# bogus2000/anytime-3D-reconstruction

Hardware: AMD Instinct MI355X
Metric: 32^3 voxel reconstructions/sec at batch=256; IoU delta vs reference (higher is better)
Workload: dtype bf16

## Files before the change

anytime-3d-reconstruction_amd/csrc/conv_direct.hip:

```cpp
#include "direct_common.h"

namespace {

constexpr int CD_CIN = 64, CD_COUT = 128;
constexpr int CD_RB = CD_CIN * 2;
constexpr int CD_PIECES = 51;
constexpr int CD_TILE = CD_PIECES * 1024;
constexpr int CD_WST = CD_COUT * 128;
constexpr int CD_NST = 3;
constexpr int CD_RING = 2 * CD_TILE;
constexpr int CD_DUMMY = CD_RING + CD_NST * CD_WST;
constexpr int CD_LDS = CD_DUMMY + 1024;
constexpr int CD_SP = CD_COUT * 2 + 16;

__global__ __launch_bounds__(512, 1) void conv_direct_kernel(const __bf16 *__restrict__ x, const __bf16 *__restrict__ w,
                                                             const float *__restrict__ scale, const float *__restrict__ shift,
                                                             void *__restrict__ y, int dout_log2, unsigned x_bytes, unsigned w_bytes,
                                                             int act, int out_fp8) {
    extern __shared__ __attribute__((aligned(16))) char smem[];
    const int tid = threadIdx.x, lane = tid & 63;
    const int wave = __builtin_amdgcn_readfirstlane(tid >> 6);
    const int wm = wave >> 1, wn = wave & 1;
    const int lo = dout_log2, no = 1 << lo, li = lo + 1, n = 1 << li;

    const VvDirectBox box = vv_direct_box(no);
    const int b = box.b, od0 = box.od0, oh0 = box.oh0, ow0 = box.ow0;

    const u32x4 rsx = vv_make_rsrc(x, x_bytes), rsw = vv_make_rsrc(w, w_bytes);
    const unsigned lds0 = (unsigned)(unsigned long long)(lptr_t)smem;

    auto issue_x = [&](int q, int slot) {
        const int piece = slot * 8 + wave;
        const int rl = piece * 8 + (lane >> 3);
        const int zd = rl / 81, rem = rl - zd * 81, jh = rem / 9, jw = rem - jh * 9;
        const int g = (lane & 7) ^ (jw & 7);
        const int id = 2 * (od0 + zd) + ((q >> 2) & 1) - 1, ih = 2 * (oh0 + jh) + ((q >> 1) & 1) - 1, iw = 2 * (ow0 + jw) + (q & 1) - 1;
// ... 156 lines not shown
    auto issue_w = [&](int c) {
        const int q = c >> 3, a = c & 7;
        const int td = 2 * ((a >> 2) & 1) + ((q >> 2) & 1), th = 2 * ((a >> 1) & 1) + ((q >> 1) & 1), tw = 2 * (a & 1) + (q & 1);
        const int t = (td * 4 + th) * 4 + tw;
        const unsigned st = lds0 + CD_RING + (c % CD_NST) * CD_WST;
#pragma unroll
        for (int i = 0; i < 2; ++i) {
            const int row = (wave * 2 + i) * 8 + (lane >> 3);
            const int g = (lane & 7) ^ ((row >> 1) & 7);
            const unsigned vo = c < 64 ? (unsigned)row * (64 * CD_RB) + t * CD_RB + g * 16 : 0xFFFFFFF0u;
            vv_dma16(rsw, vo, st + (wave * 2 + i) * 1024);
        }
    };

#pragma unroll 1
    for (int s = 0; s < 7; ++s) issue_x(0, s);
    issue_w(0);
    issue_w(1);
    issue_w(2);
    vv_wait_vm<0>();
    __syncthreads();

    const int r = lane & 15, kq = lane >> 4;
    const int rl0 = wm * 81 + (r >> 3) * 9 + (r & 7);
    unsigned xo[2][2], wo[2];
#pragma unroll
    for (int aw = 0; aw < 2; ++aw)
#pragma unroll
        for (int ks = 0; ks < 2; ++ks) xo[aw][ks] = lds0 + rl0 * CD_RB + (((ks * 4 + kq) ^ ((2 * ((r & 7) + aw)) & 7)) << 4);
#pragma unroll
    for (int ks = 0; ks < 2; ++ks) wo[ks] = lds0 + CD_RING + (wn * 64 + r) * 128 + (((ks * 4 + kq) ^ ((r >> 1) & 7)) << 4);

    f32x4 acc[4][4];
#pragma unroll
    for (int i = 0; i < 4; ++i)
#pragma unroll
        for (int j = 0; j < 4; ++j) acc[i][j] = f32x4{0.f, 0.f, 0.f, 0.f};

#define CD16_LD(F, XA, XOFF, WA)                                                                                                    \
    asm volatile("ds_read_b128 %0, %8 offset:%10\n\tds_read_b128 %1, %8 offset:%11\n\tds_read_b128 %2, %8 offset:%12\n\t"         \
                 "ds_read_b128 %3, %8 offset:%13\n\tds_read_b128 %4, %9\n\tds_read_b128 %5, %9 offset:2048\n\t"                   \
                 "ds_read_b128 %6, %9 offset:4096\n\tds_read_b128 %7, %9 offset:6144"                                               \
                 : "=&v"(F[0]), "=&v"(F[1]), "=&v"(F[2]), "=&v"(F[3]), "=&v"(F[4]), "=&v"(F[5]), "=&v"(F[6]), "=&v"(F[7])            \
                 : "v"(XA), "v"(WA), "n"(XOFF), "n"((XOFF) + 2304), "n"((XOFF) + 4608), "n"((XOFF) + 6912)                          \
                 : "memory")
#define CD16_WAIT(F, N)                                                                                                             \
    asm volatile("s_waitcnt lgkmcnt(%8)"                                                                                            \
                 : "+v"(F[0]), "+v"(F[1]), "+v"(F[2]), "+v"(F[3]), "+v"(F[4]), "+v"(F[5]), "+v"(F[6]), "+v"(F[7])                    \
                 : "n"(N)                                                                                                           \
                 : "memory")
#define CD16_SB __builtin_amdgcn_sched_barrier(0)
#define CD16_RD(D, A, OFF) asm volatile("ds_read_b128 %0, %1 offset:%2" : "=&v"(D) : "v"(A), "n"(OFF) : "memory")
#define CD16_MF(F, COT, CT)                                                                                                         \
    acc[COT][CT] = __builtin_amdgcn_mfma_f32_16x16x32_bf16(*reinterpret_cast<const bf16x8 *>(&F[4 + COT]),                          \
                                                           *reinterpret_cast<const bf16x8 *>(&F[CT]), acc[COT][CT], 0, 0, 0)

    u32x4 P[8], Q[8];
    CD16_LD(P, xo[0][0], 0, wo[0]);

#pragma unroll 1
    for (int q = 0; q < 8; ++q) {
        const unsigned tsel = (q & 1) * CD_TILE, tnext = ((q + 1) & 1) * CD_TILE;
        auto tap = [&](auto a_c) {
            constexpr int A = decltype(a_c)::value;
            constexpr int AW = A & 1, TO = (((A >> 2) & 1) * 81 + ((A >> 1) & 1) * 9 + AW) * CD_RB;
            constexpr int AN = (A + 1) & 7, AWN = AN & 1, TON = (((AN >> 2) & 1) * 81 + ((AN >> 1) & 1) * 9 + AWN) * CD_RB;
            const int c = q * 8 + A;
            const unsigned wsel = (c % CD_NST) * CD_WST, wnext = ((c + 1) % CD_NST) * CD_WST;
            const unsigned xq = xo[AW][1] + tsel, wq = wo[1] + wsel;
            CD16_WAIT(P, 0);
            CD16_SB;
            CD16_MF(P, 0, 0); CD16_MF(P, 0, 1); CD16_SB; CD16_RD(Q[0], xq, TO); CD16_RD(Q[4], wq, 0); CD16_SB;
            CD16_MF(P, 0, 2); CD16_MF(P, 0, 3); CD16_SB; CD16_RD(Q[1], xq, TO + 2304); CD16_RD(Q[5], wq, 2048); CD16_SB;
            CD16_MF(P, 1, 0); CD16_MF(P, 1, 1); CD16_SB; CD16_RD(Q[2], xq, TO + 4608); CD16_RD(Q[6], wq, 4096); CD16_SB;
            CD16_MF(P, 1, 2); CD16_MF(P, 1, 3); CD16_SB; CD16_RD(Q[3], xq, TO + 6912); CD16_RD(Q[7], wq, 6144); CD16_SB;
            CD16_MF(P, 2, 0); CD16_MF(P, 2, 1); CD16_MF(P, 2, 2); CD16_MF(P, 2, 3);
            CD16_MF(P, 3, 0); CD16_MF(P, 3, 1); CD16_MF(P, 3, 2); CD16_MF(P, 3, 3);
            CD16_SB;
            CD16_WAIT(Q, 0);
            vv_wait_vm<(A == 0 || A == 7) ? 2 : 3>();
            __syncthreads();
            CD16_SB;
            CD16_MF(Q, 0, 0); CD16_MF(Q, 0, 1);
            if (A < 7) issue_x(q + 1, A);
            CD16_MF(Q, 0, 2); CD16_MF(Q, 0, 3);
            issue_w(c + 3);
            const unsigned xp = xo[AWN][0] + (A == 7 ? tnext : tsel), wp = wo[0] + wnext;
            CD16_SB;
            CD16_MF(Q, 1, 0); CD16_MF(Q, 1, 1); CD16_SB; CD16_RD(P[0], xp, TON); CD16_RD(P[4], wp, 0); CD16_SB;
            CD16_MF(Q, 1, 2); CD16_MF(Q, 1, 3); CD16_SB; CD16_RD(P[1], xp, TON + 2304); CD16_RD(P[5], wp, 2048); CD16_SB;
            CD16_MF(Q, 2, 0); CD16_MF(Q, 2, 1); CD16_SB; CD16_RD(P[2], xp, TON + 4608); CD16_RD(P[6], wp, 4096); CD16_SB;
            CD16_MF(Q, 2, 2); CD16_MF(Q, 2, 3); CD16_SB; CD16_RD(P[3], xp, TON + 6912); CD16_RD(P[7], wp, 6144); CD16_SB;
            CD16_MF(Q, 3, 0); CD16_MF(Q, 3, 1); CD16_MF(Q, 3, 2); CD16_MF(Q, 3, 3);
            CD16_SB;
        };
        tap(std::integral_constant<int, 0>{});
        tap(std::integral_constant<int, 1>{});
        tap(std::integral_constant<int, 2>{});
        tap(std::integral_constant<int, 3>{});
        tap(std::integral_constant<int, 4>{});
        tap(std::integral_constant<int, 5>{});
        tap(std::integral_constant<int, 6>{});
        tap(std::integral_constant<int, 7>{});
    }
    CD16_WAIT(P, 0);
    vv_wait_vm<0>();
    __syncthreads();

    char *stage = smem;
    f32x4 scv[4], shv[4];
#pragma unroll
    for (int cot = 0; cot < 4; ++cot) { scv[cot] = f32x4{1.f, 1.f, 1.f, 1.f}; shv[cot] = f32x4{0.f, 0.f, 0.f, 0.f}; }
    if (scale) {
#pragma unroll
        for (int cot = 0; cot < 4; ++cot) scv[cot] = *reinterpret_cast<const f32x4 *>(scale + wn * 64 + cot * 16 + 4 * kq);
    }
    if (shift) {
#pragma unroll
        for (int cot = 0; cot < 4; ++cot) shv[cot] = *reinterpret_cast<const f32x4 *>(shift + wn * 64 + cot * 16 + 4 * kq);
    }
    auto fill = VV_DIRECT_FILL16(CD_SP, wn * 64);
    auto with_out = [&](auto act_c) {
        if (out_fp8) fill(act_c, std::true_type{});
        else fill(act_c, std::false_type{});
    };
    VV_WITH_ACT(act, with_out);
    __syncthreads();
    vv_direct_store_box<512, CD_SP, CD_COUT, CD_COUT>(stage, y, box, lo, tid, out_fp8);
}


constexpr int CDH_COUT = 64;
constexpr int CDH_WST = CDH_COUT * 128;
constexpr int CDH_RING = CD_TILE;
constexpr int CDH_DUMMY = CDH_RING + CD_NST * CDH_WST;
constexpr int CDH_LDS = CDH_DUMMY + 1024;
constexpr int CDH_SP = CDH_COUT * 2 + 16;

__global__ __launch_bounds__(256, 2) void conv_direct16h_kernel(const __bf16 *__restrict__ x, const __bf16 *__restrict__ w,
                                                                const float *__restrict__ scale, const float *__restrict__ shift,
                                                                void *__restrict__ y, int dout_log2, unsigned x_bytes, unsigned w_bytes,
                                                                int act, int out_fp8, int stagger, int abl) {
    extern __shared__ __attribute__((aligned(16))) char smem[];
    const int tid = threadIdx.x, lane = tid & 63;
// ... 50 lines not shown
    const int r = lane & 15, kq = lane >> 4;
    const int rl0 = wm * 81 + (r >> 3) * 9 + (r & 7);
    unsigned xo[2][2], wo[2];
#pragma unroll
    for (int aw = 0; aw < 2; ++aw)
#pragma unroll
        for (int ks = 0; ks < 2; ++ks) xo[aw][ks] = lds0 + rl0 * CD_RB + (((ks * 4 + kq) ^ ((2 * ((r & 7) + aw)) & 7)) << 4);
#pragma unroll
    for (int ks = 0; ks < 2; ++ks) wo[ks] = lds0 + CDH_RING + r * 128 + (((ks * 4 + kq) ^ ((r >> 1) & 7)) << 4);

    f32x4 acc[4][4];
#pragma unroll
    for (int i = 0; i < 4; ++i)
#pragma unroll
        for (int j = 0; j < 4; ++j) acc[i][j] = f32x4{0.f, 0.f, 0.f, 0.f};

    u32x4 P[8], Q[8];
#pragma unroll 1
    for (int q = 0; q < 8; ++q) {
        if (q > 0) {
            vv_wait_vm<0>();
            __syncthreads();
        }
        CD16_LD(P, xo[0][0], 0, wo[0] + ((q * 8) % CD_NST) * CDH_WST);
        auto tap = [&](auto a_c) {
            constexpr int A = decltype(a_c)::value;
            constexpr int AW = A & 1, TO = (((A >> 2) & 1) * 81 + ((A >> 1) & 1) * 9 + AW) * CD_RB;
            constexpr int AN = (A + 1) & 7, AWN = AN & 1, TON = (((AN >> 2) & 1) * 81 + ((AN >> 1) & 1) * 9 + AWN) * CD_RB;
            const int c = q * 8 + A;
            const unsigned wsel = (c % CD_NST) * CDH_WST, wnext = ((c + 1) % CD_NST) * CDH_WST;
            const unsigned xq = xo[AW][1], wq = wo[1] + wsel;
            CD16_WAIT(P, 0);
            CD16_SB;
            CD16_MF(P, 0, 0); CD16_MF(P, 0, 1); CD16_SB; CD16_RD(Q[0], xq, TO); CD16_RD(Q[4], wq, 0); CD16_SB;
            CD16_MF(P, 0, 2); CD16_MF(P, 0, 3); CD16_SB; CD16_RD(Q[1], xq, TO + 2304); CD16_RD(Q[5], wq, 2048); CD16_SB;
            CD16_MF(P, 1, 0); CD16_MF(P, 1, 1); CD16_SB; CD16_RD(Q[2], xq, TO + 4608); CD16_RD(Q[6], wq, 4096); CD16_SB;
            CD16_MF(P, 1, 2); CD16_MF(P, 1, 3); CD16_SB; CD16_RD(Q[3], xq, TO + 6912); CD16_RD(Q[7], wq, 6144); CD16_SB;
            CD16_MF(P, 2, 0); CD16_MF(P, 2, 1); CD16_MF(P, 2, 2); CD16_MF(P, 2, 3);
            CD16_MF(P, 3, 0); CD16_MF(P, 3, 1); CD16_MF(P, 3, 2); CD16_MF(P, 3, 3);
            CD16_SB;
            CD16_WAIT(Q, 0);
            vv_wait_vm<2>();
            __syncthreads();
            CD16_SB;
            CD16_MF(Q, 0, 0); CD16_MF(Q, 0, 1);
            CD16_MF(Q, 0, 2); CD16_MF(Q, 0, 3);
            issue_w(c + 3);
            CD16_SB;
            if (A < 7) {
                const unsigned xp = xo[AWN][0], wp = wo[0] + wnext;
                CD16_MF(Q, 1, 0); CD16_MF(Q, 1, 1); CD16_SB; CD16_RD(P[0], xp, TON); CD16_RD(P[4], wp, 0); CD16_SB;
                CD16_MF(Q, 1, 2); CD16_MF(Q, 1, 3); CD16_SB; CD16_RD(P[1], xp, TON + 2304); CD16_RD(P[5], wp, 2048); CD16_SB;
                CD16_MF(Q, 2, 0); CD16_MF(Q, 2, 1); CD16_SB; CD16_RD(P[2], xp, TON + 4608); CD16_RD(P[6], wp, 4096); CD16_SB;
                CD16_MF(Q, 2, 2); CD16_MF(Q, 2, 3); CD16_SB; CD16_RD(P[3], xp, TON + 6912); CD16_RD(P[7], wp, 6144); CD16_SB;
            } else {
                const bool more = q < 7 && !(abl & 1);
                CD16_MF(Q, 1, 0); CD16_MF(Q, 1, 1); CD16_SB;
                if (more) { issue_x(q + 1, 0); issue_x(q + 1, 1); issue_x(q + 1, 2); }
                CD16_SB; CD16_MF(Q, 1, 2); CD16_MF(Q, 1, 3); CD16_SB;
                if (more) { issue_x(q + 1, 3); issue_x(q + 1, 4); issue_x(q + 1, 5); }
                CD16_SB; CD16_MF(Q, 2, 0); CD16_MF(Q, 2, 1); CD16_SB;
                if (more) { issue_x(q + 1, 6); issue_x(q + 1, 7); issue_x(q + 1, 8); }
                CD16_SB; CD16_MF(Q, 2, 2); CD16_MF(Q, 2, 3); CD16_SB;
                if (more) { issue_x(q + 1, 9); issue_x(q + 1, 10); issue_x(q + 1, 11); issue_x(q + 1, 12); }
                CD16_SB;
            }
            CD16_MF(Q, 3, 0); CD16_MF(Q, 3, 1); CD16_MF(Q, 3, 2); CD16_MF(Q, 3, 3);
            CD16_SB;
        };
        tap(std::integral_constant<int, 0>{});
        tap(std::integral_constant<int, 1>{});
        tap(std::integral_constant<int, 2>{});
        tap(std::integral_constant<int, 3>{});
        tap(std::integral_constant<int, 4>{});
        tap(std::integral_constant<int, 5>{});
        tap(std::integral_constant<int, 6>{});
        tap(std::integral_constant<int, 7>{});
// ... 77 lines not shown
```

anytime-3d-reconstruction_amd/csrc/convt_whole.hip:

```cpp

#include <utility>

#include "common.h"

namespace {

constexpr int CW_X = 512 * 256;
constexpr int CW_WST = 64 * 128;
constexpr int CW_NST = 3;
constexpr int CW_RING = CW_X;
constexpr int CW_ZERO = CW_RING + CW_NST * CW_WST;
constexpr int CW_SS = CW_ZERO + 256;
constexpr int CW_LDS = CW_SS + 512;

#define CW_LD(F, X0, X1, WA)                                                                                                     \
    asm volatile("ds_read_b128 %0, %4\n\tds_read_b128 %1, %5\n\tds_read_b128 %2, %6\n\tds_read_b128 %3, %6 offset:4096"          \
                 : "=&v"(F[0]), "=&v"(F[1]), "=&v"(F[2]), "=&v"(F[3])                                                            \
                 : "v"(X0), "v"(X1), "v"(WA)                                                                                     \
                 : "memory")
#define CW_WAIT(F, N) asm volatile("s_waitcnt lgkmcnt(%4)" : "+v"(F[0]), "+v"(F[1]), "+v"(F[2]), "+v"(F[3]) : "n"(N) : "memory")
#define CW_MFMA4(F)                                                                                                              \
    do {                                                                                                                         \
        _Pragma("unroll") for (int nt = 0; nt < 2; ++nt) _Pragma("unroll") for (int mt = 0; mt < 2; ++mt)                        \
            acc[nt][mt] = __builtin_amdgcn_mfma_f32_32x32x16_bf16(*reinterpret_cast<const bf16x8 *>(&F[2 + nt]),                 \
// ... 173 lines not shown
    }
    CW_WAIT(P, 0);
    vv_wait_vm<0>();
}


#define CW16_LD(F, XA, WA)                                                                                                          \
    asm volatile("ds_read_b128 %0, %8\n\tds_read_b128 %1, %9\n\tds_read_b128 %2, %10\n\tds_read_b128 %3, %11\n\t"                    \
                 "ds_read_b128 %4, %12\n\tds_read_b128 %5, %12 offset:2048\n\tds_read_b128 %6, %12 offset:4096\n\t"                  \
                 "ds_read_b128 %7, %12 offset:6144"                                                                                 \
                 : "=&v"(F[0]), "=&v"(F[1]), "=&v"(F[2]), "=&v"(F[3]), "=&v"(F[4]), "=&v"(F[5]), "=&v"(F[6]), "=&v"(F[7])            \
                 : "v"(XA[0]), "v"(XA[1]), "v"(XA[2]), "v"(XA[3]), "v"(WA)                                                           \
                 : "memory")
#define CW16_WAIT(F, N)                                                                                                             \
    asm volatile("s_waitcnt lgkmcnt(%8)"                                                                                            \
                 : "+v"(F[0]), "+v"(F[1]), "+v"(F[2]), "+v"(F[3]), "+v"(F[4]), "+v"(F[5]), "+v"(F[6]), "+v"(F[7])                    \
                 : "n"(N)                                                                                                           \
                 : "memory")
#define CW16_SB __builtin_amdgcn_sched_barrier(0)
#define CW16_RD(D, A, OFF) asm volatile("ds_read_b128 %0, %1 offset:%2" : "=&v"(D) : "v"(A), "n"(OFF) : "memory")
#define CW16_MF(F, COT, CT)                                                                                                         \
    acc[COT][CT] = __builtin_amdgcn_mfma_f32_16x16x32_bf16(*reinterpret_cast<const bf16x8 *>(&F[4 + COT]),                          \
                                                           *reinterpret_cast<const bf16x8 *>(&F[CT]), acc[COT][CT], 0, 0, 0)

template <int ACT, bool STATS = false>
__global__ __launch_bounds__(512, 1) void ctw16_kernel(const __bf16 *__restrict__ x, const __bf16 *__restrict__ w,
                                                       const float *__restrict__ scale, const float *__restrict__ shift,
                                                       __bf16 *__restrict__ y, int npar, float *__restrict__ partial = nullptr) {
    extern __shared__ __attribute__((aligned(256))) char smem[];
    const int tid = threadIdx.x, lane = tid & 63;
    const int wave = __builtin_amdgcn_readfirstlane(tid >> 6);
    const int ps = 8 / npar;
    const int b = (int)blockIdx.x / ps, p0 = ((int)blockIdx.x % ps) * npar;
    const int NC = npar * 16;
    const unsigned lds0 = (unsigned)(unsigned long long)(lptr_t)smem;

    const u32x4 rsx = vv_make_rsrc(x + (size_t)b * (512 * 128), CW_X);
    const u32x4 rsw = vv_make_rsrc(w, 64 * 128 * 64 * 2);
    {
        const int pos = lane & 15, vsub = lane >> 4;
#pragma unroll 1
        for (int i = 0; i < 16; ++i) {
            const int it = i * 8 + wave;
            const int v = it * 4 + vsub;
            vv_dma16(rsx, (unsigned)(v * 256 + ((pos ^ ((2 * v) & 15)) << 4)), lds0 + it * 1024);
        }
    }
    const unsigned wv = (unsigned)((wave * 8 + (lane >> 3)) * 128 + (((lane & 7) ^ (((wave * 8 + (lane >> 3)) >> 1) & 7)) << 4));
    auto issue_w = [&](int c, int s) {
        const int cc = c < NC ? c : NC - 1;
        const unsigned soff = (unsigned)__builtin_amdgcn_readfirstlane((p0 * 16 + cc) * CW_WST);
        vv_dma16(rsw, wv, soff, lds0 + CW_RING + s * CW_WST + wave * 1024);
    };
    issue_w(0, 0);
    issue_w(1, 1);
    issue_w(2, 2);
    if (tid < 16) *reinterpret_cast<uint4 *>(smem + CW_ZERO + tid * 16) = uint4{0u, 0u, 0u, 0u};
    if (tid >= 64 && tid < 128) {
        const int ch = tid - 64;
        *reinterpret_cast<float *>(smem + CW_SS + ch * 4) = scale ? scale[ch] : 1.f;
        *reinterpret_cast<float *>(smem + CW_SS + 256 + ch * 4) = shift ? shift[ch] : 0.f;
    }
    vv_wait_vm<0>();
    __syncthreads();

    const int r = lane & 15, q = lane >> 4;
    const int rh = r >> 3, rw = r & 7;
    const unsigned wl = lds0 + CW_RING + r * 128 + ((q ^ ((r >> 1) & 7)) << 4);
    const unsigned R0 = lds0 + (unsigned)((wave * 64 + r) << 8);
    const unsigned ZR = lds0 + CW_ZERO;
    auto tap_setup = [&](auto a_c, int pd, int ph, int pw, unsigned (&t)[4]) {
        constexpr int A = decltype(a_c)::value;
        const int dd = pd - ((A >> 2) & 1), dh = ph - ((A >> 1) & 1), dw = pw - (A & 1);
        const bool okw = (unsigned)(wave + dd) < 8u && (unsigned)(rw + dw) < 8u;
        const int sft = dd * 64 + dh * 8 + dw;
        const unsigned key = ((unsigned)((2 * (rw + dw)) ^ q) & 15u) << 4;
#pragma unroll
        for (int ct = 0; ct < 4; ++ct) {
            const unsigned row = okw && (unsigned)(2 * ct + rh + dh) < 8u ? R0 + (unsigned)((sft + 16 * ct) << 8) : ZR;
            t[ct] = row ^ key;
        }
    };

    f32x4 acc[4][4];
#pragma unroll
    for (int i = 0; i < 4; ++i)
#pragma unroll
        for (int j = 0; j < 4; ++j) acc[i][j] = f32x4{0.f, 0.f, 0.f, 0.f};
    f32x4 st1[4], st2[4];
#pragma unroll
    for (int i = 0; i < 4; ++i) { st1[i] = f32x4{0.f, 0.f, 0.f, 0.f}; st2[i] = f32x4{0.f, 0.f, 0.f, 0.f}; }

    auto epilogue = [&](int p) {
        const int pd = (p >> 2) & 1, ph = (p >> 1) & 1, pw = p & 1;
        const int qo = (q & 1) * 32 + (q >> 1) * 16;
        char *yb = reinterpret_cast<char *>(y) + ((((size_t)b * 16 + 2 * wave + pd) * 16 + 2 * rh + ph) * 16 + 2 * rw + pw) * 128 + qo;
        const char *ss = smem + CW_SS + q * 16;
#pragma unroll
        for (int c2 = 0; c2 < 2; ++c2) {
            u32x2 o[2][4];
#pragma unroll
            for (int h = 0; h < 2; ++h) {
                const int cot = 2 * c2 + h;
                const f32x4 sc = *reinterpret_cast<const f32x4 *>(ss + cot * 64);
                const f32x4 sh = *reinterpret_cast<const f32x4 *>(ss + 256 + cot * 64);
#pragma unroll
                for (int ct = 0; ct < 4; ++ct) {
                    const f32x4 t = vv_bn_act4<ACT>(acc[cot][ct], sc, sh);
                    bf16x4 v;
#pragma unroll
                    for (int e = 0; e < 4; ++e) v[e] = static_cast<__bf16>(t[e]);
                    if (STATS) {
                        const f32x4 f = {(float)v[0], (float)v[1], (float)v[2], (float)v[3]};
                        st1[cot] += f;
                        st2[cot] += f * f;
                    }
                    acc[cot][ct] = f32x4{0.f, 0.f, 0.f, 0.f};
                    o[h][ct] = *reinterpret_cast<const u32x2 *>(&v);
                }
            }
#pragma unroll
            for (int ct = 0; ct < 4; ++ct) {
                auto rx = __builtin_amdgcn_permlane16_swap(o[0][ct][0], o[1][ct][0], false, false);
                auto ry = __builtin_amdgcn_permlane16_swap(o[0][ct][1], o[1][ct][1], false, false);
                *reinterpret_cast<u32x4 *>(yb + (size_t)(ct * 4 * 16 * 128) + c2 * 64) = u32x4{rx[0], ry[0], rx[1], ry[1]};
            }
        }
    };

    u32x4 P[8], Q[8];
    unsigned ua[4], ub[4];
    tap_setup(std::integral_constant<int, 0>{}, (p0 >> 2) & 1, (p0 >> 1) & 1, p0 & 1, ua);
    unsigned ws = wl;
    int stg = 0, cw = 3;
    CW16_LD(P, ua, ws);
#pragma unroll 1
    for (int pi = 0; pi < npar; ++pi) {
        const int p = p0 + pi, pd = (p >> 2) & 1, ph = (p >> 1) & 1, pw = p & 1;
        const int pn = p + 1, pnd = (pn >> 2) & 1, pnh = (pn >> 1) & 1, pnw = pn & 1;
        auto chunk = [&](auto j_c) {
            constexpr int J = decltype(j_c)::value, A = J >> 1, KH = J & 1;
            unsigned xq[4];
#pragma unroll
            for (int ct = 0; ct < 4; ++ct) xq[ct] = ua[ct] ^ (KH ? 192u : 64u);
            const unsigned wq = ws ^ 64u;
            CW16_WAIT(P, 0);
            CW16_SB;
            CW16_MF(P, 0, 0); CW16_MF(P, 0, 1); CW16_SB; CW16_RD(Q[0], xq[0], 0); CW16_RD(Q[4], wq, 0); CW16_SB;
            CW16_MF(P, 0, 2); CW16_MF(P, 0, 3); CW16_SB; CW16_RD(Q[1], xq[1], 0); CW16_RD(Q[5], wq, 2048); CW16_SB;
            CW16_MF(P, 1, 0); CW16_MF(P, 1, 1); CW16_SB; CW16_RD(Q[2], xq[2], 0); CW16_RD(Q[6], wq, 4096); CW16_SB;
            CW16_MF(P, 1, 2); CW16_MF(P, 1, 3); CW16_SB; CW16_RD(Q[3], xq[3], 0); CW16_RD(Q[7], wq, 6144); CW16_SB;
            CW16_MF(P, 2, 0); CW16_MF(P, 2, 1); CW16_MF(P, 2, 2); CW16_MF(P, 2, 3);
            if (KH == 0) {
                if (A < 7) tap_setup(std::integral_constant<int, (A + 1) & 7>{}, pd, ph, pw, ub);
                else tap_setup(std::integral_constant<int, 0>{}, pnd, pnh, pnw, ub);
            }
            CW16_MF(P, 3, 0); CW16_MF(P, 3, 1); CW16_MF(P, 3, 2); CW16_MF(P, 3, 3);
            CW16_SB;
            CW16_WAIT(Q, 0);
            if (J < 2 && pi > 0) vv_wait_vm<9>();
            else vv_wait_vm<1>();
            __builtin_amdgcn_s_barrier();
            CW16_SB;
            CW16_MF(Q, 0, 0); CW16_MF(Q, 0, 1); CW16_SB;
            issue_w(cw, stg);
            ++cw;
            stg = stg == CW_NST - 1 ? 0 : stg + 1;
            ws = wl + stg * CW_WST;
            if (KH == 0) {
#pragma unroll
                for (int ct = 0; ct < 4; ++ct) xq[ct] = ua[ct] ^ 128u;
            } else {
#pragma unroll
                for (int ct = 0; ct < 4; ++ct) xq[ct] = ua[ct] = ub[ct];
            }
            CW16_SB;
            CW16_MF(Q, 0, 2); CW16_MF(Q, 0, 3); CW16_SB; CW16_RD(P[0], xq[0], 0); CW16_RD(P[4], ws, 0); CW16_SB;
            CW16_MF(Q, 1, 0); CW16_MF(Q, 1, 1); CW16_SB; CW16_RD(P[1], xq[1], 0); CW16_RD(P[5], ws, 2048); CW16_SB;
            CW16_MF(Q, 1, 2); CW16_MF(Q, 1, 3); CW16_SB; CW16_RD(P[2], xq[2], 0); CW16_RD(P[6], ws, 4096); CW16_SB;
            CW16_MF(Q, 2, 0); CW16_MF(Q, 2, 1); CW16_SB; CW16_RD(P[3], xq[3], 0); CW16_RD(P[7], ws, 6144); CW16_SB;
            CW16_MF(Q, 2, 2); CW16_MF(Q, 2, 3);
            CW16_MF(Q, 3, 0); CW16_MF(Q, 3, 1); CW16_MF(Q, 3, 2); CW16_MF(Q, 3, 3);
            CW16_SB;
        };
        chunk(std::integral_constant<int, 0>{});
        chunk(std::integral_constant<int, 1>{});
        chunk(std::integral_constant<int, 2>{});
        chunk(std::integral_constant<int, 3>{});
        chunk(std::integral_constant<int, 4>{});
        chunk(std::integral_constant<int, 5>{});
        chunk(std::integral_constant<int, 6>{});
        chunk(std::integral_constant<int, 7>{});
        chunk(std::integral_constant<int, 8>{});
        chunk(std::integral_constant<int, 9>{});
        chunk(std::integral_constant<int, 10>{});
        chunk(std::integral_constant<int, 11>{});
        chunk(std::integral_constant<int, 12>{});
        chunk(std::integral_constant<int, 13>{});
        chunk(std::integral_constant<int, 14>{});
        chunk(std::integral_constant<int, 15>{});
        epilogue(p);
    }
    CW16_WAIT(P, 0);
    vv_wait_vm<0>();
    if (STATS) {
#pragma unroll
        for (int cot = 0; cot < 4; ++cot)
#pragma unroll
            for (int e = 0; e < 4; ++e) {
                float a = st1[cot][e], b2 = st2[cot][e];
#pragma unroll
                for (int o = 8; o > 0; o >>= 1) { a += __shfl_xor(a, o, 64); b2 += __shfl_xor(b2, o, 64); }
                st1[cot][e] = a; st2[cot][e] = b2;
            }
        __syncthreads();
        float *red = reinterpret_cast<float *>(smem);
        if (r == 0) {
#pragma unroll
            for (int cot = 0; cot < 4; ++cot) {
                *reinterpret_cast<f32x4 *>(red + (wave * 2 + 0) * 64 + 16 * cot + 4 * q) = st1[cot];
                *reinterpret_cast<f32x4 *>(red + (wave * 2 + 1) * 64 + 16 * cot + 4 * q) = st2[cot];
            }
        }
        __syncthreads();
// ... 351 lines not shown
```

anytime-3d-reconstruction_amd/csrc/direct_common.h:

```cpp
#pragma once
#include "common.h"

struct VvDirectBox { int b, od0, oh0, ow0, nh; };

template <bool HALVES = false>
__device__ __forceinline__ VvDirectBox vv_direct_box(int no) {
    const int nwg = gridDim.x;
    int blk = (nwg & 7) == 0 ? (int)(blockIdx.x & 7) * (nwg >> 3) + (int)(blockIdx.x >> 3) : (int)blockIdx.x;
    VvDirectBox o;
    o.nh = 0;
    if (HALVES) { o.nh = blk & 1; blk >>= 1; }
    const int bxw = no >> 3, bxh = no >> 3, bxd = no >> 2;
    const int bw = blk % bxw; blk /= bxw;
    const int bh = blk % bxh; blk /= bxh;
    const int bd = blk % bxd;
    o.b = blk / bxd;
    o.od0 = bd * 4; o.oh0 = bh * 8; o.ow0 = bw * 8;
    return o;
}

#define VV_DIRECT_PUT4(dst, c, v)                                                                          \
    do {                                                                                                   \
        if (FP8) {                                                                                         \
            *reinterpret_cast<unsigned *>(dst + c) = vv_pack_fp8x4(v);                                     \
        } else {                                                                                           \
            bf16x4 o;                                                                                      \
            _Pragma("unroll") for (int e = 0; e < 4; ++e) o[e] = static_cast<__bf16>(v[e]);                \
            *reinterpret_cast<bf16x4 *>(dst + c * 2) = o;                                                  \
        }                                                                                                  \
    } while (0)

#define VV_DIRECT_FILL16(PITCH, C0)                                                                        \
    [&](auto act_c, auto fp8_c) {                                                                          \
        constexpr int ACT = decltype(act_c)::value;                                                        \
        constexpr bool FP8 = decltype(fp8_c)::value;                                                       \
        _Pragma("unroll") for (int ct = 0; ct < 4; ++ct)                                                   \
            _Pragma("unroll") for (int cot = 0; cot < 4; ++cot) {                                          \
                const int c = (C0) + cot * 16 + 4 * kq;                                                    \
                const f32x4 sc = scv[cot], sh = shv[cot];                                                  \
                const f32x4 v = vv_bn_act4<ACT>(acc[cot][ct], sc, sh);                                     \
                char *dst = stage + (wm * 64 + ct * 16 + r) * (PITCH);                                     \
                VV_DIRECT_PUT4(dst, c, v);                                                                 \
            }                                                                                              \
    }
#define VV_DIRECT_FILL32(PITCH, C0)                                                                        \
    [&](auto act_c, auto fp8_c) {                                                                          \
        constexpr int ACT = decltype(act_c)::value;                                                        \
        constexpr bool FP8 = decltype(fp8_c)::value;                                                       \
        _Pragma("unroll") for (int mt = 0; mt < 2; ++mt)                                                   \
            _Pragma("unroll") for (int nt = 0; nt < 2; ++nt)                                               \
                _Pragma("unroll") for (int g = 0; g < 4; ++g) {                                            \
                    const int c = (C0) + nt * 32 + 8 * g + 4 * fh;                                         \
                    const f32x4 sc = scv[nt][g], sh = shv[nt][g];                                          \
                    f32x4 v;                                                                               \
                    _Pragma("unroll") for (int e = 0; e < 4; ++e) {                                        \
                        float t = acc[nt][mt][4 * g + e] * sc[e] + sh[e];                                  \
                        if (ACT == VV_ACT_ELU) { const float em = __expf(fminf(t, 0.f)) - 1.f; t = t > 0.f ? t : em; } \
                        else if (ACT == VV_ACT_RELU) t = fmaxf(t, 0.f);                                    \
                        else if (ACT == VV_ACT_LRELU) t = t > 0.f ? t : 0.3f * t;                          \
                        v[e] = t;                                                                          \
                    }                                                                                      \
                    char *dst = stage + (wm * 64 + mt * 32 + fr) * (PITCH);                                \
                    VV_DIRECT_PUT4(dst, c, v);                                                             \
                }                                                                                          \
    }

template <int THREADS, int PITCH, int STAGE_CH, int Y_CH>
// ... 12 lines not shown
```

Baseline: 571,700.

## Skip MFMAs on zero-padded depth taps in direct conv and transposed conv

Both kernels' tile-to-wave mappings are remapped so each MFMA column tile corresponds to one depth plane, not a mix of rows. Boundary blocks (first/last depth slab, or a given dz half) can then drop the MFMA for the padded plane at compile time, using a SKIP template parameter through specialised phase/parity loops. The direct conv LDS read strides and the epilogue staging fill are changed to match the new layout, and the transposed conv output addressing is updated to match. This adds code size from the extra specialised loop copies and changes the LDS access pattern, which may affect bank conflicts. A microbenchmark script is also added.

```diff
diff --git a/anytime-3d-reconstruction_amd/csrc/conv_direct.hip b/anytime-3d-reconstruction_amd/csrc/conv_direct.hip
--- a/anytime-3d-reconstruction_amd/csrc/conv_direct.hip
+++ b/anytime-3d-reconstruction_amd/csrc/conv_direct.hip
@@ -12,6 +12,8 @@
 constexpr int CD_DUMMY = CD_RING + CD_NST * CD_WST;
 constexpr int CD_LDS = CD_DUMMY + 1024;
 constexpr int CD_SP = CD_COUT * 2 + 16;
+constexpr int CD16_PL = 81 * CD_RB;
+constexpr int CD16_HP = 18 * CD_RB;
 
 __global__ __launch_bounds__(512, 1) void conv_direct_kernel(const __bf16 *__restrict__ x, const __bf16 *__restrict__ w,
                                                              const float *__restrict__ scale, const float *__restrict__ shift,
@@ -214,7 +216,7 @@
     __syncthreads();
 
     const int r = lane & 15, kq = lane >> 4;
-    const int rl0 = wm * 81 + (r >> 3) * 9 + (r & 7);
+    const int rl0 = wm * 18 + (r >> 3) * 9 + (r & 7);
     unsigned xo[2][2], wo[2];
 #pragma unroll
     for (int aw = 0; aw < 2; ++aw)
@@ -229,12 +231,12 @@
 #pragma unroll
         for (int j = 0; j < 4; ++j) acc[i][j] = f32x4{0.f, 0.f, 0.f, 0.f};
 
-#define CD16_LD(F, XA, XOFF, WA)                                                                                                    \
+#define CD16_LD(F, XA, XOFF, WA, STEP)                                                                                                \
     asm volatile("ds_read_b128 %0, %8 offset:%10\n\tds_read_b128 %1, %8 offset:%11\n\tds_read_b128 %2, %8 offset:%12\n\t"         \
                  "ds_read_b128 %3, %8 offset:%13\n\tds_read_b128 %4, %9\n\tds_read_b128 %5, %9 offset:2048\n\t"                   \
                  "ds_read_b128 %6, %9 offset:4096\n\tds_read_b128 %7, %9 offset:6144"                                               \
                  : "=&v"(F[0]), "=&v"(F[1]), "=&v"(F[2]), "=&v"(F[3]), "=&v"(F[4]), "=&v"(F[5]), "=&v"(F[6]), "=&v"(F[7])            \
-                 : "v"(XA), "v"(WA), "n"(XOFF), "n"((XOFF) + 2304), "n"((XOFF) + 4608), "n"((XOFF) + 6912)                          \
+                 : "v"(XA), "v"(WA), "n"(XOFF), "n"((XOFF) + (STEP)), "n"((XOFF) + 2 * (STEP)), "n"((XOFF) + 3 * (STEP))                      \
                  : "memory")
 #define CD16_WAIT(F, N)                                                                                                             \
     asm volatile("s_waitcnt lgkmcnt(%8)"                                                                                            \
@@ -246,15 +248,20 @@
 #define CD16_MF(F, COT, CT)                                                                                                         \
     acc[COT][CT] = __builtin_amdgcn_mfma_f32_16x16x32_bf16(*reinterpret_cast<const bf16x8 *>(&F[4 + COT]),                          \
                                                            *reinterpret_cast<const bf16x8 *>(&F[CT]), acc[COT][CT], 0, 0, 0)
+#define CD16_MFS(F, COT, CT)                                                                                                        \
+    do {                                                                                                                            \
+        if constexpr ((CT) != SKIP) CD16_MF(F, COT, CT);                                                                            \
+    } while (0)
 
     u32x4 P[8], Q[8];
-    CD16_LD(P, xo[0][0], 0, wo[0]);
-
+    CD16_LD(P, xo[0][0], 0, wo[0], CD16_PL);
+
+    auto phases = [&](int qb, int qe, auto lo_c, auto hi_c) {
 #pragma unroll 1
-    for (int q = 0; q < 8; ++q) {
+    for (int q = qb; q < qe; ++q) {
         const unsigned tsel = (q & 1) * CD_TILE, tnext = ((q + 1) & 1) * CD_TILE;
-        auto tap = [&](auto a_c) {
-            constexpr int A = decltype(a_c)::value;
+        auto tap = [&](auto a_c, auto skip_c) {
+            constexpr int A = decltype(a_c)::value, SKIP = decltype(skip_c)::value;
             constexpr int AW = A & 1, TO = (((A >> 2) & 1) * 81 + ((A >> 1) & 1) * 9 + AW) * CD_RB;
             constexpr int AN = (A + 1) & 7, AWN = AN & 1, TON = (((AN >> 2) & 1) * 81 + ((AN >> 1) & 1) * 9 + AWN) * CD_RB;
             const int c = q * 8 + A;
@@ -262,39 +269,45 @@
             const unsigned xq = xo[AW][1] + tsel, wq = wo[1] + wsel;
             CD16_WAIT(P, 0);
             CD16_SB;
-            CD16_MF(P, 0, 0); CD16_MF(P, 0, 1); CD16_SB; CD16_RD(Q[0], xq, TO); CD16_RD(Q[4], wq, 0); CD16_SB;
-            CD16_MF(P, 0, 2); CD16_MF(P, 0, 3); CD16_SB; CD16_RD(Q[1], xq, TO + 2304); CD16_RD(Q[5], wq, 2048); CD16_SB;
-            CD16_MF(P, 1, 0); CD16_MF(P, 1, 1); CD16_SB; CD16_RD(Q[2], xq, TO + 4608); CD16_RD(Q[6], wq, 4096); CD16_SB;
-            CD16_MF(P, 1, 2); CD16_MF(P, 1, 3); CD16_SB; CD16_RD(Q[3], xq, TO + 6912); CD16_RD(Q[7], wq, 6144); CD16_SB;
-            CD16_MF(P, 2, 0); CD16_MF(P, 2, 1); CD16_MF(P, 2, 2); CD16_MF(P, 2, 3);
-            CD16_MF(P, 3, 0); CD16_MF(P, 3, 1); CD16_MF(P, 3, 2); CD16_MF(P, 3, 3);
+            CD16_MFS(P, 0, 0); CD16_MFS(P, 0, 1); CD16_SB; CD16_RD(Q[0], xq, TO); CD16_RD(Q[4], wq, 0); CD16_SB;
+            CD16_MFS(P, 0, 2); CD16_MFS(P, 0, 3); CD16_SB; CD16_RD(Q[1], xq, TO + CD16_PL); CD16_RD(Q[5], wq, 2048); CD16_SB;
+            CD16_MFS(P, 1, 0); CD16_MFS(P, 1, 1); CD16_SB; CD16_RD(Q[2], xq, TO + 2 * CD16_PL); CD16_RD(Q[6], wq, 4096); CD16_SB;
+            CD16_MFS(P, 1, 2); CD16_MFS(P, 1, 3); CD16_SB; CD16_RD(Q[3], xq, TO + 3 * CD16_PL); CD16_RD(Q[7], wq, 6144); CD16_SB;
+            CD16_MFS(P, 2, 0); CD16_MFS(P, 2, 1); CD16_MFS(P, 2, 2); CD16_MFS(P, 2, 3);
+            CD16_MFS(P, 3, 0); CD16_MFS(P, 3, 1); CD16_MFS(P, 3, 2); CD16_MFS(P, 3, 3);
             CD16_SB;
             CD16_WAIT(Q, 0);
             vv_wait_vm<(A == 0 || A == 7) ? 2 : 3>();
             __syncthreads();
             CD16_SB;
-            CD16_MF(Q, 0, 0); CD16_MF(Q, 0, 1);
+            CD16_MFS(Q, 0, 0); CD16_MFS(Q, 0, 1);
             if (A < 7) issue_x(q + 1, A);
-            CD16_MF(Q, 0, 2); CD16_MF(Q, 0, 3);
+            CD16_MFS(Q, 0, 2); CD16_MFS(Q, 0, 3);
             issue_w(c + 3);
             const unsigned xp = xo[AWN][0] + (A == 7 ? tnext : tsel), wp = wo[0] + wnext;
             CD16_SB;
-            CD16_MF(Q, 1, 0); CD16_MF(Q, 1, 1); CD16_SB; CD16_RD(P[0], xp, TON); CD16_RD(P[4], wp, 0); CD16_SB;
-            CD16_MF(Q, 1, 2); CD16_MF(Q, 1, 3); CD16_SB; CD16_RD(P[1], xp, TON + 2304); CD16_RD(P[5], wp, 2048); CD16_SB;
-            CD16_MF(Q, 2, 0); CD16_MF(Q, 2, 1); CD16_SB; CD16_RD(P[2], xp, TON + 4608); CD16_RD(P[6], wp, 4096); CD16_SB;
-            CD16_MF(Q, 2, 2); CD16_MF(Q, 2, 3); CD16_SB; CD16_RD(P[3], xp, TON + 6912); CD16_RD(P[7], wp, 6144); CD16_SB;
-            CD16_MF(Q, 3, 0); CD16_MF(Q, 3, 1); CD16_MF(Q, 3, 2); CD16_MF(Q, 3, 3);
+            CD16_MFS(Q, 1, 0); CD16_MFS(Q, 1, 1); CD16_SB; CD16_RD(P[0], xp, TON); CD16_RD(P[4], wp, 0); CD16_SB;
+            CD16_MFS(Q, 1, 2); CD16_MFS(Q, 1, 3); CD16_SB; CD16_RD(P[1], xp, TON + CD16_PL); CD16_RD(P[5], wp, 2048); CD16_SB;
+            CD16_MFS(Q, 2, 0); CD16_MFS(Q, 2, 1); CD16_SB; CD16_RD(P[2], xp, TON + 2 * CD16_PL); CD16_RD(P[6], wp, 4096); CD16_SB;
+            CD16_MFS(Q, 2, 2); CD16_MFS(Q, 2, 3); CD16_SB; CD16_RD(P[3], xp, TON + 3 * CD16_PL); CD16_RD(P[7], wp, 6144); CD16_SB;
+            CD16_MFS(Q, 3, 0); CD16_MFS(Q, 3, 1); CD16_MFS(Q, 3, 2); CD16_MFS(Q, 3, 3);
             CD16_SB;
         };
-        tap(std::integral_constant<int, 0>{});
-        tap(std::integral_constant<int, 1>{});
-        tap(std::integral_constant<int, 2>{});
-        tap(std::integral_constant<int, 3>{});
-        tap(std::integral_constant<int, 4>{});
-        tap(std::integral_constant<int, 5>{});
-        tap(std::integral_constant<int, 6>{});
-        tap(std::integral_constant<int, 7>{});
-    }
+        tap(std::integral_constant<int, 0>{}, lo_c);
+        tap(std::integral_constant<int, 1>{}, lo_c);
+        tap(std::integral_constant<int, 2>{}, lo_c);
+        tap(std::integral_constant<int, 3>{}, lo_c);
+        tap(std::integral_constant<int, 4>{}, hi_c);
+        tap(std::integral_constant<int, 5>{}, hi_c);
+        tap(std::integral_constant<int, 6>{}, hi_c);
+        tap(std::integral_constant<int, 7>{}, hi_c);
+    }
+    };
+    constexpr std::integral_constant<int, -1> none{};
+    const bool first = od0 == 0, last = od0 + 4 == no;
+    if (first) phases(0, 4, std::integral_constant<int, 0>{}, none);
+    phases(first ? 4 : 0, last ? 4 : 8, none, none);
+    if (last) phases(4, 8, none, std::integral_constant<int, 3>{});
     CD16_WAIT(P, 0);
     vv_wait_vm<0>();
     __syncthreads();
@@ -311,7 +324,7 @@
 #pragma unroll
         for (int cot = 0; cot < 4; ++cot) shv[cot] = *reinterpret_cast<const f32x4 *>(shift + wn * 64 + cot * 16 + 4 * kq);
     }
-    auto fill = VV_DIRECT_FILL16(CD_SP, wn * 64);
+    auto fill = VV_DIRECT_FILL16P(CD_SP, wn * 64);
     auto with_out = [&](auto act_c) {
         if (out_fp8) fill(act_c, std::true_type{});
         else fill(act_c, std::false_type{});
@@ -408,7 +421,7 @@
             vv_wait_vm<0>();
             __syncthreads();
         }
-        CD16_LD(P, xo[0][0], 0, wo[0] + ((q * 8) % CD_NST) * CDH_WST);
+        CD16_LD(P, xo[0][0], 0, wo[0] + ((q * 8) % CD_NST) * CDH_WST, CD16_HP);
         auto tap = [&](auto a_c) {
             constexpr int A = decltype(a_c)::value;
             constexpr int AW = A & 1, TO = (((A >> 2) & 1) * 81 + ((A >> 1) & 1) * 9 + AW) * CD_RB;
@@ -419,9 +432,9 @@
             CD16_WAIT(P, 0);
             CD16_SB;
             CD16_MF(P, 0, 0); CD16_MF(P, 0, 1); CD16_SB; CD16_RD(Q[0], xq, TO); CD16_RD(Q[4], wq, 0); CD16_SB;
-            CD16_MF(P, 0, 2); CD16_MF(P, 0, 3); CD16_SB; CD16_RD(Q[1], xq, TO + 2304); CD16_RD(Q[5], wq, 2048); CD16_SB;
-            CD16_MF(P, 1, 0); CD16_MF(P, 1, 1); CD16_SB; CD16_RD(Q[2], xq, TO + 4608); CD16_RD(Q[6], wq, 4096); CD16_SB;
-            CD16_MF(P, 1, 2); CD16_MF(P, 1, 3); CD16_SB; CD16_RD(Q[3], xq, TO + 6912); CD16_RD(Q[7], wq, 6144); CD16_SB;
+            CD16_MF(P, 0, 2); CD16_MF(P, 0, 3); CD16_SB; CD16_RD(Q[1], xq, TO + CD16_HP); CD16_RD(Q[5], wq, 2048); CD16_SB;
+            CD16_MF(P, 1, 0); CD16_MF(P, 1, 1); CD16_SB; CD16_RD(Q[2], xq, TO + 2 * CD16_HP); CD16_RD(Q[6], wq, 4096); CD16_SB;
+            CD16_MF(P, 1, 2); CD16_MF(P, 1, 3); CD16_SB; CD16_RD(Q[3], xq, TO + 3 * CD16_HP); CD16_RD(Q[7], wq, 6144); CD16_SB;
             CD16_MF(P, 2, 0); CD16_MF(P, 2, 1); CD16_MF(P, 2, 2); CD16_MF(P, 2, 3);
             CD16_MF(P, 3, 0); CD16_MF(P, 3, 1); CD16_MF(P, 3, 2); CD16_MF(P, 3, 3);
             CD16_SB;
@@ -436,9 +449,9 @@
             if (A < 7) {
                 const unsigned xp = xo[AWN][0], wp = wo[0] + wnext;
                 CD16_MF(Q, 1, 0); CD16_MF(Q, 1, 1); CD16_SB; CD16_RD(P[0], xp, TON); CD16_RD(P[4], wp, 0); CD16_SB;
-                CD16_MF(Q, 1, 2); CD16_MF(Q, 1, 3); CD16_SB; CD16_RD(P[1], xp, TON + 2304); CD16_RD(P[5], wp, 2048); CD16_SB;
-                CD16_MF(Q, 2, 0); CD16_MF(Q, 2, 1); CD16_SB; CD16_RD(P[2], xp, TON + 4608); CD16_RD(P[6], wp, 4096); CD16_SB;
-                CD16_MF(Q, 2, 2); CD16_MF(Q, 2, 3); CD16_SB; CD16_RD(P[3], xp, TON + 6912); CD16_RD(P[7], wp, 6144); CD16_SB;
+                CD16_MF(Q, 1, 2); CD16_MF(Q, 1, 3); CD16_SB; CD16_RD(P[1], xp, TON + CD16_HP); CD16_RD(P[5], wp, 2048); CD16_SB;
+                CD16_MF(Q, 2, 0); CD16_MF(Q, 2, 1); CD16_SB; CD16_RD(P[2], xp, TON + 2 * CD16_HP); CD16_RD(P[6], wp, 4096); CD16_SB;
+                CD16_MF(Q, 2, 2); CD16_MF(Q, 2, 3); CD16_SB; CD16_RD(P[3], xp, TON + 3 * CD16_HP); CD16_RD(P[7], wp, 6144); CD16_SB;
             } else {
                 const bool more = q < 7 && !(abl & 1);
                 CD16_MF(Q, 1, 0); CD16_MF(Q, 1, 1); CD16_SB;
diff --git a/anytime-3d-reconstruction_amd/csrc/convt_whole.hip b/anytime-3d-reconstruction_amd/csrc/convt_whole.hip
--- a/anytime-3d-reconstruction_amd/csrc/convt_whole.hip
+++ b/anytime-3d-reconstruction_amd/csrc/convt_whole.hip
@@ -219,6 +219,10 @@
 #define CW16_MF(F, COT, CT)                                                                                                         \
     acc[COT][CT] = __builtin_amdgcn_mfma_f32_16x16x32_bf16(*reinterpret_cast<const bf16x8 *>(&F[4 + COT]),                          \
                                                            *reinterpret_cast<const bf16x8 *>(&F[CT]), acc[COT][CT], 0, 0, 0)
+#define CW16_MFS(F, COT, CT)                                                                                                        \
+    do {                                                                                                                            \
+        if constexpr ((CT) != SKIP) CW16_MF(F, COT, CT);                                                                            \
+    } while (0)
 
 template <int ACT, bool STATS = false>
 __global__ __launch_bounds__(512, 1) void ctw16_kernel(const __bf16 *__restrict__ x, const __bf16 *__restrict__ w,
@@ -264,17 +268,18 @@
     const int r = lane & 15, q = lane >> 4;
     const int rh = r >> 3, rw = r & 7;
     const unsigned wl = lds0 + CW_RING + r * 128 + ((q ^ ((r >> 1) & 7)) << 4);
-    const unsigned R0 = lds0 + (unsigned)((wave * 64 + r) << 8);
+    const int hp = wave & 3, dz = wave >> 2;
+    const unsigned R0 = lds0 + (unsigned)((dz * 256 + hp * 16 + r) << 8);
     const unsigned ZR = lds0 + CW_ZERO;
     auto tap_setup = [&](auto a_c, int pd, int ph, int pw, unsigned (&t)[4]) {
         constexpr int A = decltype(a_c)::value;
         const int dd = pd - ((A >> 2) & 1), dh = ph - ((A >> 1) & 1), dw = pw - (A & 1);
-        const bool okw = (unsigned)(wave + dd) < 8u && (unsigned)(rw + dw) < 8u;
+        const bool okw = (unsigned)(2 * hp + rh + dh) < 8u && (unsigned)(rw + dw) < 8u;
         const int sft = dd * 64 + dh * 8 + dw;
         const unsigned key = ((unsigned)((2 * (rw + dw)) ^ q) & 15u) << 4;
 #pragma unroll
         for (int ct = 0; ct < 4; ++ct) {
-            const unsigned row = okw && (unsigned)(2 * ct + rh + dh) < 8u ? R0 + (unsigned)((sft + 16 * ct) << 8) : ZR;
+            const unsigned row = okw && (unsigned)(4 * dz + ct + dd) < 8u ? R0 + (unsigned)((sft + 64 * ct) << 8) : ZR;
             t[ct] = row ^ key;
         }
     };
@@ -291,7 +296,7 @@
     auto epilogue = [&](int p) {
         const int pd = (p >> 2) & 1, ph = (p >> 1) & 1, pw = p & 1;
         const int qo = (q & 1) * 32 + (q >> 1) * 16;
-        char *yb = reinterpret_cast<char *>(y) + ((((size_t)b * 16 + 2 * wave + pd) * 16 + 2 * rh + ph) * 16 + 2 * rw + pw) * 128 + qo;
+        char *yb = reinterpret_cast<char *>(y) + ((((size_t)b * 16 + 8 * dz + pd) * 16 + 2 * (2 * hp + rh) + ph) * 16 + 2 * rw + pw) * 128 + qo;
         const char *ss = smem + CW_SS + q * 16;
 #pragma unroll
         for (int c2 = 0; c2 < 2; ++c2) {
@@ -320,7 +325,7 @@
             for (int ct = 0; ct < 4; ++ct) {
                 auto rx = __builtin_amdgcn_permlane16_swap(o[0][ct][0], o[1][ct][0], false, false);
                 auto ry = __builtin_amdgcn_permlane16_swap(o[0][ct][1], o[1][ct][1], false, false);
-                *reinterpret_cast<u32x4 *>(yb + (size_t)(ct * 4 * 16 * 128) + c2 * 64) = u32x4{rx[0], ry[0], rx[1], ry[1]};
+                *reinterpret_cast<u32x4 *>(yb + (size_t)(ct * 2 * 16 * 16 * 128) + c2 * 64) = u32x4{rx[0], ry[0], rx[1], ry[1]};
             }
         }
     };
@@ -331,35 +336,37 @@
     unsigned ws = wl;
     int stg = 0, cw = 3;
     CW16_LD(P, ua, ws);
+    auto parities = [&](int pb, int pe, auto lo_c, auto hi_c) {
+    constexpr int LO = decltype(lo_c)::value, HI = decltype(hi_c)::value;
 #pragma unroll 1
-    for (int pi = 0; pi < npar; ++pi) {
-        const int p = p0 + pi, pd = (p >> 2) & 1, ph = (p >> 1) & 1, pw = p & 1;
+    for (int p = pb; p < pe; ++p) {
+        const int pi = p - p0, pd = (p >> 2) & 1, ph = (p >> 1) & 1, pw = p & 1;
         const int pn = p + 1, pnd = (pn >> 2) & 1, pnh = (pn >> 1) & 1, pnw = pn & 1;
         auto chunk = [&](auto j_c) {
-            constexpr int J = decltype(j_c)::value, A = J >> 1, KH = J & 1;
+            constexpr int J = decltype(j_c)::value, A = J >> 1, KH = J & 1, SKIP = J < 8 ? LO : HI;
             unsigned xq[4];
 #pragma unroll
             for (int ct = 0; ct < 4; ++ct) xq[ct] = ua[ct] ^ (KH ? 192u : 64u);
             const unsigned wq = ws ^ 64u;
             CW16_WAIT(P, 0);
             CW16_SB;
-            CW16_MF(P, 0, 0); CW16_MF(P, 0, 1); CW16_SB; CW16_RD(Q[0], xq[0], 0); CW16_RD(Q[4], wq, 0); CW16_SB;
-            CW16_MF(P, 0, 2); CW16_MF(P, 0, 3); CW16_SB; CW16_RD(Q[1], xq[1], 0); CW16_RD(Q[5], wq, 2048); CW16_SB;
-            CW16_MF(P, 1, 0); CW16_MF(P, 1, 1); CW16_SB; CW16_RD(Q[2], xq[2], 0); CW16_RD(Q[6], wq, 4096); CW16_SB;
-            CW16_MF(P, 1, 2); CW16_MF(P, 1, 3); CW16_SB; CW16_RD(Q[3], xq[3], 0); CW16_RD(Q[7], wq, 6144); CW16_SB;
-            CW16_MF(P, 2, 0); CW16_MF(P, 2, 1); CW16_MF(P, 2, 2); CW16_MF(P, 2, 3);
+            CW16_MFS(P, 0, 0); CW16_MFS(P, 0, 1); CW16_SB; CW16_RD(Q[0], xq[0], 0); CW16_RD(Q[4], wq, 0); CW16_SB;
+            CW16_MFS(P, 0, 2); CW16_MFS(P, 0, 3); CW16_SB; CW16_RD(Q[1], xq[1], 0); CW16_RD(Q[5], wq, 2048); CW16_SB;
+            CW16_MFS(P, 1, 0); CW16_MFS(P, 1, 1); CW16_SB; CW16_RD(Q[2], xq[2], 0); CW16_RD(Q[6], wq, 4096); CW16_SB;
+            CW16_MFS(P, 1, 2); CW16_MFS(P, 1, 3); CW16_SB; CW16_RD(Q[3], xq[3], 0); CW16_RD(Q[7], wq, 6144); CW16_SB;
+            CW16_MFS(P, 2, 0); CW16_MFS(P, 2, 1); CW16_MFS(P, 2, 2); CW16_MFS(P, 2, 3);
             if (KH == 0) {
                 if (A < 7) tap_setup(std::integral_constant<int, (A + 1) & 7>{}, pd, ph, pw, ub);
                 else tap_setup(std::integral_constant<int, 0>{}, pnd, pnh, pnw, ub);
             }
-            CW16_MF(P, 3, 0); CW16_MF(P, 3, 1); CW16_MF(P, 3, 2); CW16_MF(P, 3, 3);
+            CW16_MFS(P, 3, 0); CW16_MFS(P, 3, 1); CW16_MFS(P, 3, 2); CW16_MFS(P, 3, 3);
             CW16_SB;
             CW16_WAIT(Q, 0);
             if (J < 2 && pi > 0) vv_wait_vm<9>();
             else vv_wait_vm<1>();
             __builtin_amdgcn_s_barrier();
             CW16_SB;
-            CW16_MF(Q, 0, 0); CW16_MF(Q, 0, 1); CW16_SB;
+            CW16_MFS(Q, 0, 0); CW16_MFS(Q, 0, 1); CW16_SB;
             issue_w(cw, stg);
             ++cw;
             stg = stg == CW_NST - 1 ? 0 : stg + 1;
@@ -372,12 +379,12 @@
                 for (int ct = 0; ct < 4; ++ct) xq[ct] = ua[ct] = ub[ct];
             }
             CW16_SB;
-            CW16_MF(Q, 0, 2); CW16_MF(Q, 0, 3); CW16_SB; CW16_RD(P[0], xq[0], 0); CW16_RD(P[4], ws, 0); CW16_SB;
-            CW16_MF(Q, 1, 0); CW16_MF(Q, 1, 1); CW16_SB; CW16_RD(P[1], xq[1], 0); CW16_RD(P[5], ws, 2048); CW16_SB;
-            CW16_MF(Q, 1, 2); CW16_MF(Q, 1, 3); CW16_SB; CW16_RD(P[2], xq[2], 0); CW16_RD(P[6], ws, 4096); CW16_SB;
-            CW16_MF(Q, 2, 0); CW16_MF(Q, 2, 1); CW16_SB; CW16_RD(P[3], xq[3], 0); CW16_RD(P[7], ws, 6144); CW16_SB;
-            CW16_MF(Q, 2, 2); CW16_MF(Q, 2, 3);
-            CW16_MF(Q, 3, 0); CW16_MF(Q, 3, 1); CW16_MF(Q, 3, 2); CW16_MF(Q, 3, 3);
+            CW16_MFS(Q, 0, 2); CW16_MFS(Q, 0, 3); CW16_SB; CW16_RD(P[0], xq[0], 0); CW16_RD(P[4], ws, 0); CW16_SB;
+            CW16_MFS(Q, 1, 0); CW16_MFS(Q, 1, 1); CW16_SB; CW16_RD(P[1], xq[1], 0); CW16_RD(P[5], ws, 2048); CW16_SB;
+            CW16_MFS(Q, 1, 2); CW16_MFS(Q, 1, 3); CW16_SB; CW16_RD(P[2], xq[2], 0); CW16_RD(P[6], ws, 4096); CW16_SB;
+            CW16_MFS(Q, 2, 0); CW16_MFS(Q, 2, 1); CW16_SB; CW16_RD(P[3], xq[3], 0); CW16_RD(P[7], ws, 6144); CW16_SB;
+            CW16_MFS(Q, 2, 2); CW16_MFS(Q, 2, 3);
+            CW16_MFS(Q, 3, 0); CW16_MFS(Q, 3, 1); CW16_MFS(Q, 3, 2); CW16_MFS(Q, 3, 3);
             CW16_SB;
         };
         chunk(std::integral_constant<int, 0>{});
@@ -397,6 +404,14 @@
         chunk(std::integral_constant<int, 14>{});
         chunk(std::integral_constant<int, 15>{});
         epilogue(p);
+    }
+    };
+    {
+        constexpr std::integral_constant<int, -1> none{};
+        const int pe = p0 + npar, p4 = p0 > 4 ? p0 : 4, e4 = pe < 4 ? pe : 4;
+        if (dz == 0) parities(p0, e4, none, std::integral_constant<int, 0>{});
+        parities(dz == 0 ? p4 : p0, dz == 0 ? pe : e4, none, none);
+        if (dz != 0) parities(p4, pe, std::integral_constant<int, 3>{}, none);
     }
     CW16_WAIT(P, 0);
     vv_wait_vm<0>();
diff --git a/anytime-3d-reconstruction_amd/csrc/direct_common.h b/anytime-3d-reconstruction_amd/csrc/direct_common.h
--- a/anytime-3d-reconstruction_amd/csrc/direct_common.h
+++ b/anytime-3d-reconstruction_amd/csrc/direct_common.h
@@ -43,6 +43,19 @@
                 VV_DIRECT_PUT4(dst, c, v);                                                                 \
             }                                                                                              \
     }
+#define VV_DIRECT_FILL16P(PITCH, C0)                                                                       \
+    [&](auto act_c, auto fp8_c) {                                                                          \
+        constexpr int ACT = decltype(act_c)::value;                                                        \
+        constexpr bool FP8 = decltype(fp8_c)::value;                                                       \
+        _Pragma("unroll") for (int ct = 0; ct < 4; ++ct)                                                   \
+            _Pragma("unroll") for (int cot = 0; cot < 4; ++cot) {                                          \
+                const int c = (C0) + cot * 16 + 4 * kq;                                                    \
+                const f32x4 sc = scv[cot], sh = shv[cot];                                                  \
+                const f32x4 v = vv_bn_act4<ACT>(acc[cot][ct], sc, sh);                                     \
+                char *dst = stage + (ct * 64 + wm * 16 + r) * (PITCH);                                     \
+                VV_DIRECT_PUT4(dst, c, v);                                                                 \
+            }                                                                                              \
+    }
 #define VV_DIRECT_FILL32(PITCH, C0)                                                                        \
     [&](auto act_c, auto fp8_c) {                                                                          \
         constexpr int ACT = decltype(act_c)::value;                                                        \
diff --git a/profiles/microbench/mb_dpad_skip.py b/profiles/microbench/mb_dpad_skip.py
--- /dev/null
+++ b/profiles/microbench/mb_dpad_skip.py
@@ -0,0 +1,68 @@
+import ctypes, json, os, statistics, sys
+import torch
+_R = os.path.dirname(os.path.dirname(os.path.dirname(os.path.abspath(__file__)))); sys.path.insert(0, _R); sys.path.insert(0, os.path.join(_R, 'anytime-3d-reconstruction_amd'))
+from voxvae import lib as L
+out_path = sys.argv[1]
+libs = {}
+for a in sys.argv[2:]:
+    name, path = a.split('=', 1)
+    libs[name] = ctypes.CDLL(os.path.join(_R, path))
+base = next(iter(libs))
+L.load()
+DEV = 'cuda:0'; B = 256
+ALT, WARM, N = int(os.environ.get('MB_ALT', 9)), 20, 60
+cs = ctypes.c_void_p(torch.cuda.current_stream().cuda_stream)
+torch.manual_seed(0)
+sc = torch.rand(256, device=DEV) + 0.5; sh = torch.randn(256, device=DEV) * 0.3
+
+
+def packed(fn, wshape, cin, cout, *extra):
+    w = (torch.randn(*wshape, device=DEV) / (8 * cin) ** 0.5).float().contiguous()
+    o = torch.empty(64 * cin * cout, dtype=torch.bfloat16, device=DEV)
+    L.call(fn, L.ptr(w), L.ptr(o), cin, cout, *extra, cs)
+    return o
+
+
+w2 = packed('vv_pack_conv_k4', (4, 4, 4, 64, 128), 64, 128, L.VV_BF16)
+x2 = torch.randn(B, 16, 16, 16, 64, device=DEV).to(torch.bfloat16)
+w4 = packed('vv_pack_convT_k4s2_skip', (4, 4, 4, 64, 128), 128, 64)
+x4 = torch.randn(B, 8, 8, 8, 128, device=DEV).to(torch.bfloat16)
+cases = {
+    'E2': ('vv_conv3d_k4s2_direct_fwd', lambda y: (L.ptr(x2), L.ptr(w2), L.ptr(sc), L.ptr(sh), L.ptr(y), B, 16, 64, 128, 1, L.VV_BF16, cs), (B, 8, 8, 8, 128)),
+    'D4': ('vv_convT3d_k4s2_whole_fwd', lambda y: (L.ptr(x4), L.ptr(w4), L.ptr(sc), L.ptr(sh), L.ptr(y), B, 8, 128, 64, 1, L.VV_BF16, cs), (B, 16, 16, 16, 64)),
+}
+res = {'batch': B, 'alternations': ALT, 'launches_per_alternation': N, 'timer': 'hipEvent pair around each launch', 'baseline': base}
+for name, (fn, args, oshape) in cases.items():
+    ys = {k: torch.full(oshape, float('nan'), dtype=torch.bfloat16, device=DEV) for k in libs}
+    fs = {}
+    for k in libs:
+        f = getattr(libs[k], fn); f.restype = ctypes.c_int
+        fs[k] = f
+        assert f(*args(ys[k])) == 0
+    torch.cuda.synchronize()
+    same = {k: bool(torch.equal(ys[k].view(torch.int16), ys[base].view(torch.int16))) for k in libs}
+    equal = {k: bool((ys[k].float() == ys[base].float()).all()) for k in libs}
+    med = {k: [] for k in libs}
+    for alt in range(ALT):
+        for k in libs:
+            a = args(ys[k])
+            for _ in range(WARM):
+                fs[k](*a)
+            ev = [(torch.cuda.Event(enable_timing=True), torch.cuda.Event(enable_timing=True)) for _ in range(N)]
+            for e0, e1 in ev:
+                e0.record()
+                fs[k](*a)
+                e1.record()
+            torch.cuda.synchronize()
+            med[k].append(statistics.median(1e3 * e0.elapsed_time(e1) for e0, e1 in ev))
+    r = {}
+    for k in libs:
+        m = statistics.median(med[k])
+        r[k] = {'us_median': round(m, 2), 'us_min': round(min(med[k]), 2), 'us_max': round(max(med[k]), 2),
+                'alternation_medians_us': [round(v, 2) for v in med[k]], 'bytes_identical_to_baseline': same[k], 'equal_to_baseline': equal[k]}
+    for k in libs:
+        r[k]['over_baseline'] = round(r[k]['us_median'] / r[base]['us_median'], 4)
+    res[name] = r
+    print(json.dumps({name: r}), flush=True)
+with open(os.path.join(_R, out_path), 'w') as f:
+    json.dump(res, f, indent=1)
```

Result: no change. 575,900, median of 6 (+0.7%).
